# HyTruongSon/GraphFlow

Measured on AMD Instinct MI355X. Metric: CCN-2D (SMP_omega) molecules/sec fwd+bwd, higher is better.
Workload: dtype f32 (level block products: 2xf16-split operands, 22-bit, fp32 accumulate); 1 GPU; cfg3: SMP_omega 3 levels, C=64, F=5, D=5, cap=29, batch=1024 synthetic QM9-size molecules/GPU, device-resident, fused levels; parallelism=single GPU

## Files before the change

graphflow_amd/_lib.py:

```python
import ctypes as C
import os
import subprocess

_CSRC = os.path.join(os.path.dirname(os.path.abspath(__file__)), "csrc")
LIB_PATH = os.environ.get("GF_HIP_LIBRARY") or os.path.join(_CSRC, "libgf_hip.so")

GF_OK, GF_ERR_INVALID, GF_ERR_HIP, GF_ERR_NOMEM, GF_ERR_UNSUPPORTED, GF_ERR_TIMEOUT = range(6)
GF_OPT_R18_GENERIC_KERNELS = 1
GF_OPT_SMP_FP32_PRODUCTS = 2
GF_DIST_ID_BYTES = 128

_fp = C.POINTER(C.c_float)
_dp = C.POINTER(C.c_double)
_vp = C.c_void_p

PROTOTYPES = {
    "gf_ctx_create": (C.c_int, [C.POINTER(_vp), C.c_int, _vp]),
    "gf_ctx_use_private_stream": (C.c_int, [_vp]),
    "gf_ctx_destroy": (C.c_int, [_vp]),
    "gf_ctx_set_stream": (C.c_int, [_vp, _vp]),
    "gf_ctx_get_stream": (_vp, [_vp]),
    "gf_ctx_synchronize": (C.c_int, [_vp]),
    "gf_ctx_reserve": (C.c_int, [_vp, C.c_size_t]),
    "gf_ctx_set_timing": (C.c_int, [_vp, C.c_int]),
# ... 70 lines not shown
    "gf_smp_parameters_upload": (_i, [_vp, _fp]),
    "gf_smp_parameters_download": (_i, [_vp, _fp, _fp]),
    "gf_smp_forward_host": (_i, [_vp, _dp, _dp, _dp, _dp]),
    "gf_smp_adam_step": (_i, [_vp, _vp, _vp, C.c_double, _i]),
    "gf_smp_adam_reset": (_i, [_vp]),
    "gf_smp_momentum_step": (_i, [_vp, _vp, _vp, C.c_double, _i, C.c_double]),
    "gf_smp_uniform_init_host": (_i, [_vp, _fp]),
    "gf_smp_save_model": (_i, [_vp, _vp, C.c_char_p]),
    "gf_smp_load_model": (_i, [_vp, _vp, C.c_char_p]),
    "gf_smp_set_fused": (_i, [_vp, _i]),
    "gf_smp_device_bytes": (_i, [_vp, _vp, _vp]),
    "gf_smp_level_products_f32": (_i, [_vp, _i, _i, _vp, _vp, _vp, _vp, _vp]),
    "gf_smp_level_wgrad_f32": (_i, [_vp, _i, _vp, _vp, _vp, _vp, _vp]),
    "gf_smp_level_products_ex_f32": (_i, [_vp, _i, _i, _i, _i, _i, _vp, _vp, _vp, _vp, _vp, _vp, _i, _vp]),
    "gf_smp_level_wgrad_ex_f32": (_i, [_vp, _i, _i, _i, _i, _vp, _vp, _vp, _vp, _vp, _vp, _vp]),
    "gf_smp_prepare_molecule_host": (_i, [_vp, _i, C.POINTER(C.c_int), _dp, C.POINTER(C.c_int), _dp]),
    "gf_smp_receptive_field": (_i, [_vp, _i, _i, _i, C.POINTER(C.c_int), _i]),
    "gf_smp_read_activation": (C.c_longlong, [_vp, _i, _i, _i, _vp, C.c_size_t]),
    "gf_smp_read_reduced_adjacency": (C.c_longlong, [_vp, _i, _i, _i, _vp, C.c_size_t]),
    "gf_smp_level_sizes": (_i, [_vp, _i, C.POINTER(C.c_longlong), C.POINTER(C.c_longlong), C.POINTER(C.c_longlong)]),
    "gf_smp_level_present_rows": (C.c_longlong, [_vp, _i]),
    "gf_smp_level_pairs": (C.c_longlong, [_vp, _i]),
    "gf_smp_level_covered_rows": (C.c_longlong, [_vp, _i]),
    "gf_stack_forward_f32": (_i, [_vp, _vp, _vp, _i, C.c_size_t]),
    "gf_stack_backward_f32": (_i, [_vp, _vp, _vp, _i, C.c_size_t]),
})

PROTOTYPES.update({
    "gf_smp_dropout_masks": (_i, [_vp, _vp, C.c_float]),
    "gf_adam_step_f32": (_i, [_vp, _vp, _vp, _vp, _vp, C.c_size_t, C.c_double, _i, C.c_ulonglong]),
# ... 40 lines not shown
```

graphflow_amd/csrc/smp_fused.hip:

```cpp
#include <algorithm>
#include <type_traits>

#include "r18_device.h"
#include "smp_internal.h"

using namespace gf::dev;

namespace gf {
namespace {

__device__ __forceinline__ f4 fold_two_tables(f4 u, f4 v) {
    f4 z;
#pragma unroll
    for (int k = 0; k < 4; ++k) {
        const auto r = __builtin_amdgcn_permlane16_swap(__float_as_uint(u[k]), __float_as_uint(v[k]), false, false);
        z[k] = xor32_sum(__uint_as_float(r[0]) + __uint_as_float(r[1]));
    }
    return z;
}

__device__ __forceinline__ f4 dpp_xor8(f4 v) {
    f4 r;
#pragma unroll
    for (int k = 0; k < 4; ++k)
// ... 1423 lines not shown
    }
    const int ocols = smp_compact_o(s) ? 2 : O_COLS;
    const int ldt = T_COLS * C, ldo = O_COLS * C;
    {
        const long long tC = C, wCC = (long long)CC;
        GemmSpec sp[3] = {
            {T, d.Wst, O + O_LOC * C, rows, C, 5 * C, ldt, C, ldo, 3, {T_SAB * tC, T_SAB * tC, T_T6 * tC, 0}, {0 * wCC, 2 * wCC, 3 * wCC, 0},
             {2 * C, C, 2 * C, 0}, d.rowscale, 2, {0, 1, -1, -1}},
            {T + T_SAB * C, d.Wst + 5 * CC, O + O_Z * C, rows, C, 2 * C, ldt, C, ldo, 0, {0, 0, 0, 0}, {0, 0, 0, 0}, {0, 0, 0, 0}, nullptr, 0,
             {-1, -1, -1, -1}},
            {T + T_SAB * C, d.Wst + 7 * CC, O + O_ZP * C, rows, C, C, ldt, C, ldo, 0, {0, 0, 0, 0}, {0, 0, 0, 0}, {0, 0, 0, 0}, nullptr, 0,
             {-1, -1, -1, -1}},
        };
        if (smp_c64_kernels(s)) {
            st = smp_rowpanel_products_c64(ctx, true, T, drop ? d.rowfac8 : d.rowscale, d.Wst, O, rows, d.trow, d.trowf, false,
                                           d.wimg_ready ? d.wimg : nullptr, C, drop ? 8 : 2, smp_extras_in_kernel(s, l) ? 3 : 0);
            if (st != GF_OK) return st;
        } else if (gemm_grouped_supported(sp, 3, false, false)) {
            st = gemm_grouped_rows(ctx, false, false, sp, 3, rows);
            if (st != GF_OK) return st;
        } else {
            struct G { int tcol, kb, wpos, ocol, scol, acc; };
            const G gs[5] = {{T_SAB, 2, 0, O_LOC, 0, 0}, {T_SAB, 1, 2, O_LOC, 1, 1}, {T_T6, 2, 3, O_LOC, -1, 1},
                             {T_SAB, 2, 5, O_Z, -1, 0}, {T_SAB, 1, 7, O_ZP, -1, 0}};
            for (const G &g : gs) {
                st = gemm_rs(ctx, false, false, rows, C, g.kb * C, T + g.tcol * C, ldt, 0, d.Wst + g.wpos * CC, C, 0, O + g.ocol * C, ldo,
                             0, 1, g.acc, d.rowscale, 2, g.scol);
                if (st != GF_OK) return st;
            }
        }
    }
// ... 217 lines not shown
        fa.splits[g] = grp[g]->splits;
        fa.n[g] = (unsigned)grp[g]->n;
        fa.first[g] = firsts[g];
    }
    fa.part[5] = colpart;
    fa.splits[5] = nb;
    fa.n[5] = (unsigned)C;
    fa.first[5] = firsts[5];
    const unsigned total = (unsigned)(18 * CC + C);
    GF_LAUNCH(ctx, "smpf_fold", smp_fold_level, dim3((total + 63) / 64), dim3(256), 0, fa, dKl, dbl, C, s->cfg.custom_matmul, total);
    st = smp_dp_level_done(s, l);
    if (st != GF_OK) return st;
    if (d.fwd_c64) {
        st = smp_rowpanel_products_c64(ctx, false, dO, drop ? d.rowfac8 : d.rowscale, d.Wst, dT, rows, ocols == 2 ? d.trow : nullptr, d.trowf,
                                       smp_fused_gather_enabled(s, l), d.wimg_ready ? d.wimg : nullptr, C, drop ? 8 : 2,
                                       (ocols == 2 && smp_extras_in_kernel(s, l)) ? 3 : 0);
        x_bwd_done = ocols == 2 && smp_extras_in_kernel(s, l);
        if (st != GF_OK) return st;
    } else {
        const long long oC = C, wCC = (long long)CC;
        GemmSpec dg[3] = {
            {dO, d.Wst, dT + T_SAB * C, rows, C, 4 * C, ldo, C, ldt, 4, {O_LOC * oC, O_LOC * oC, O_Z * oC, O_ZP * oC},
             {0 * wCC, 2 * wCC, 5 * wCC, 7 * wCC}, {C, C, C, C}, d.rowscale, 2, {0, 1, -1, -1}},
            {dO, d.Wst, dT + T_SBC * C, rows, C, 2 * C, ldo, C, ldt, 2, {O_LOC * oC, O_Z * oC, 0, 0}, {1 * wCC, 6 * wCC, 0, 0}, {C, C, 0, 0},
             d.rowscale, 2, {0, -1, -1, -1}},
            {dO, d.Wst, dT + T_T6 * C, rows, 2 * C, C, ldo, C, ldt, 1, {O_LOC * oC, 0, 0, 0}, {3 * wCC, 0, 0, 0}, {C, 0, 0, 0}, nullptr, 0,
             {-1, -1, -1, -1}},
        };
        if (gemm_grouped_supported(dg, 3, false, true)) {
            st = gemm_grouped_rows(ctx, false, true, dg, 3, rows);
            if (st != GF_OK) return st;
// ... 187 lines not shown
```

graphflow_amd/csrc/smp_internal.h:

```cpp
#ifndef GF_SMP_INTERNAL_H_INCLUDED
#define GF_SMP_INTERNAL_H_INCLUDED

#include <vector>

#include "gf_internal.h"
#include "smp_prep.h"

namespace gf {
gf_status gemm(gf_ctx *ctx, bool ta, bool tb, int M, int N, int K, const float *A, int lda, long long sA, const float *B,
               int ldb, long long sB, float *C, int ldc, long long sC, int batch, int accumulate);
gf_status gemm_rs(gf_ctx *ctx, bool ta, bool tb, int M, int N, int K, const float *A, int lda, long long sA, const float *B,
                  int ldb, long long sB, float *C, int ldc, long long sC, int batch, int accumulate, const float *rs,
                  int rs_ld, int scol);
struct GemmSpec {
    const float *A, *B;
    float *C;
    int M, N, K, lda, ldb, ldc;
    int nseg;
    long long a_off[4], b_off[4];
    int klen[4];
    const float *rs;
    int rs_ld;
    int scol[4];
};
struct FoldGroup {
    const float *part;
    int splits;
    size_t n;
};
gf_status gemm_grouped_free(gf_ctx *ctx, bool tb, const GemmSpec *specs, int n, const char *name);
gf_status gemm_grouped_free_tn(gf_ctx *ctx, const GemmSpec *specs, int n, float *part, size_t part_floats, FoldGroup *out,
                               const char *name);
bool gemm_grouped_supported(const GemmSpec *specs, int n, bool ta, bool tb);
gf_status gemm_grouped_rows(gf_ctx *ctx, bool ta, bool tb, const GemmSpec *specs, int n, int rows, int accumulate = 0);
gf_status gemm_grouped_splitk(gf_ctx *ctx, const GemmSpec *specs, int n, int rows, float *dest, int accumulate);
gf_status smp_rowpanel_products_c64(gf_ctx *ctx, bool forward, const float *A, const float *rowscale, const float *Wst, float *Out,
                                    int rows, const int *trow, const int *trowf = nullptr, bool skip_zero_grads = false,
                                    const void *wimg = nullptr, int C = 64,
                                    int nf = 2, int nx = 0);
bool smp_split_products(const gf_ctx *ctx);
gf_status smp_rowpanel_split_c64(gf_ctx *ctx, bool forward, const float *A, const float *rowscale, const float *Wst, float *Out,
                                 int rows, const int *trow, int cus, const int *trowf = nullptr, bool skip_zero_grads = false,
                                 const void *wimg = nullptr, int C = 64, int nf = 2, int nx = 0);
size_t smp_split_image_bytes();
gf_status smp_split_build_images(gf_ctx *ctx, const float *const *Wst, void *const *img, int n, int C = 64, const float *const *X = nullptr);
gf_status smp_wgrad_partials_all(gf_ctx *ctx, const float *T, const float *dO, const float *rowscale, int rows, int splits, float *part,
                                 const int *trow, const int *trowf, unsigned *words, const unsigned *chan = nullptr, float smax = 0.f,
                                 const unsigned *row_max = nullptr, int nf = 2, int C = 32, float *xpart = nullptr);
gf_status smp_wgrad_channel_maxima_ld(gf_ctx *ctx, const float *fprev, long long prev_rows, int ld0, const float *dsrc, long long drows, int ld1, int C,
                                      unsigned *words);
size_t smp_wgrad_all_words();
int smp_wgrad_all_splits(gf_ctx *ctx, long long rows);
gf_status smp_small_split_c64(gf_ctx *ctx, bool transposed, int n, const int *prog, const float *const *In, float *const *Out, const int *rows,
                              const int *pos0, const void *wimg, const char *name, int C = 64);
struct WgradScales {
    const unsigned *cmax = nullptr, *chan = nullptr;
    float smax = 0.f, max_tot = 0.f, max_tr = 0.f;
    const unsigned *row_max = nullptr;
// ... 71 lines not shown
        int4 *tf_recs = nullptr;
        float *psum = nullptr;
        float *dshl = nullptr;
        bool psum_ready = false;
        float *pmax = nullptr;
        float *dzmax = nullptr;
        long long dz_rows = 0;
        int dz_ld = 64;
        long long dz_rows2 = 0, dz_off2 = 0;
        int dz_ld2 = 64;
        bool pmax_ready = false;
        void *wimg = nullptr;
        bool wimg_ready = false;
        bool fwd_c64 = false;
        int *trowf = nullptr;
        float max_tot = 0.f, max_tr = 0.f;
        const unsigned *row_max = nullptr;
        long long *pair_src_pair = nullptr, *cons_row = nullptr, *cons_pair = nullptr;
        int *node_center = nullptr, *cons_a = nullptr, *mol_order = nullptr, *gather_items = nullptr;
        float *Fdc = nullptr, *Gc = nullptr, *dGc = nullptr, *dFdc = nullptr;
        float *f = nullptr, *df = nullptr, *Q = nullptr;
        float *sh = nullptr, *vf = nullptr;
        int *node_of_vertex = nullptr, *node_mol = nullptr;
        int *node_present = nullptr;
        int *field = nullptr;
        unsigned *keep_mask = nullptr;
        float *nodefac = nullptr, *rowfac8 = nullptr;
        float *Vt = nullptr, *dVt = nullptr;
        float *St = nullptr, *dSt = nullptr;
        float *scal = nullptr;
// ... 121 lines not shown
```

graphflow_amd/csrc/smp_level_c64.hip:

```cpp
#include <algorithm>
#include <cstdlib>

#include "gemm_lds.h"
#include "gf_internal.h"
#include "smp_internal.h"

namespace gf {
namespace {

using namespace lds_image;

constexpr int kWgThreads = 1024, kWgARows = 256, kWgBRows = 192;
constexpr int kWgStage = (kWgARows + kWgBRows) * LDS_ROW + 2 * BK;
__constant__ int c_wg_ablk[8] = {0, 1, 0, 2, 3, 0, 1, 0};
__constant__ int c_wg_bblk[8] = {0, 0, 0, 0, 0, 1, 1, 2};
__constant__ int c_wg_scale[8] = {0, 0, 1, -1, -1, -1, -1, -1};

__global__ __launch_bounds__(kWgThreads, 1) void smp_wgrad_c64(const float *__restrict__ T, const float *__restrict__ dO,
                                                               const float *__restrict__ rs, int rows, int kchunk,
                                                               float *__restrict__ part, const int *__restrict__ trow) {
    extern __shared__ __attribute__((aligned(16))) float wg_smem[];
    const int tid = threadIdx.x, lane = tid & 63, li = lane & 31, lh = lane >> 5;
    const int wave = __builtin_amdgcn_readfirstlane(tid >> 6);
    const int prod = wave >> 1, nh = wave & 1;
// ... 350 lines not shown
    if (kchunk < 8 * BK) kchunk = 8 * BK;
    const int splits = (rows + kchunk - 1) / kchunk;
    if ((size_t)splits * total > part_floats)
        return fail(ctx, GF_ERR_NOMEM, "smp_wgrad_partials_c64: %d partial images, room for %zu", splits, part_floats / total);
    out->splits = splits;
    if (trow && ws.any() && smp_split_products(ctx))
        return smp_wgrad_partials_split_c64(ctx, T, dO, rowscale, rows, kchunk, splits, part, trow, ws, trowf);
    const size_t lds = sizeof(float) * 2 * (size_t)kWgStage;
    gf_status st = opt_in_lds(ctx, smp_wgrad_c64, lds);
    if (st != GF_OK) return st;
    GF_LAUNCH(ctx, "smpf_wgrad", smp_wgrad_c64, dim3((unsigned)splits), dim3(kWgThreads), lds, T, dO, rowscale, rows, kchunk, part, trow);
    return GF_OK;
}

gf_status smp_rowpanel_products_c64(gf_ctx *ctx, bool forward, const float *A, const float *rowscale, const float *Wst, float *Out,
                                    int rows, const int *trow, const int *trowf, bool skip_zero_grads, const void *wimg, int C, int nf, int nx) {
    if (rows < 1) return GF_OK;
    static int cu_count[64] = {};
    const int di = ctx->device & 63;
    if (!cu_count[di]) {
        GF_HIP_TRY(ctx, hipDeviceGetAttribute(&cu_count[di], hipDeviceAttributeMultiprocessorCount, ctx->device));
        if (cu_count[di] < 1) cu_count[di] = 256;
    }
    const int cus = cu_count[di];
    if (trow && smp_split_products(ctx)) return smp_rowpanel_split_c64(ctx, forward, A, rowscale, Wst, Out, rows, trow, cus, trowf, skip_zero_grads, wimg, C, nf, nx);
    if (C != 64 || nf != 2 || nx != 0) return fail(ctx, GF_ERR_UNSUPPORTED, "smp_rowpanel_products: %d channels / %d row factors / %d extra products on the fp32 matrix pipe", C, nf, nx);
    const size_t lds = sizeof(float) * 8 * 2 * 2 * 32 * (size_t)kRpWRow;
    const int th = (forward && !trow) ? 1024 : 512;
    const int npanels = (rows + 31) / 32, per = th / 64;
    const int want = (npanels + per - 1) / per;
    const int grid = want < cus ? want : cus;
    const char *name = forward ? "smpf_products_fwd" : "smpf_products_bwd";
#define GF_RP_LAUNCH(F, T, Cm)                                                                                              \
    do {                                                                                                                    \
        gf_status st__ = opt_in_lds(ctx, smp_rowpanel_c64<F, T, Cm>, lds);                                                  \
        if (st__ != GF_OK) return st__;                                                                                     \
        GF_LAUNCH(ctx, name, (smp_rowpanel_c64<F, T, Cm>), dim3((unsigned)grid), dim3(T), lds, A, rowscale, Wst, Out, rows, trow); \
    } while (0)
    if (trow) {
        if (forward) GF_RP_LAUNCH(true, 512, true);
// ... 12 lines not shown
```

graphflow_amd/csrc/smp_level_c64_split.hip:

```cpp
#include <cstdlib>
#include <type_traits>

#include "gemm_lds.h"
#include "gf_internal.h"
#include "smp_internal.h"

namespace gf {
namespace {

using lds_image::f16v;
using lds_image::f4v;
typedef _Float16 h8 __attribute__((ext_vector_type(8)));
typedef _Float16 h2 __attribute__((ext_vector_type(2)));
typedef float f2v __attribute__((ext_vector_type(2)));

constexpr int kSpThreads = 512;

template <unsigned EMIN = 14u>
__device__ __forceinline__ void pow2_scale(unsigned maxbits, float *s, float *inv) {
    unsigned e = maxbits >> 23;
    e = e < EMIN ? EMIN : e;
    *s = __uint_as_float((267u - e) << 23);
    *inv = __uint_as_float((e - 13u) << 23);
}
// ... 81 lines not shown
        if (blockIdx.x == 0)
            build_weight_images<true, 1, 16>(w, H, L, winv, wmax, threadIdx.x);
        else
            build_weight_images<false, 1, 16>(w, H, L, winv, wmax, threadIdx.x);
    } else {
        if (blockIdx.x == 0)
            build_weight_images<true, 1, 32>(w, H, L, winv, wmax, threadIdx.x);
        else
            build_weight_images<false, 1, 32>(w, H, L, winv, wmax, threadIdx.x);
    }
}

#ifndef GF_SP_WHOLE_PANEL
#define GF_SP_WHOLE_PANEL 16
#endif
template <bool FWD, bool MASK, int CB = 64, int NF = 2, int NX = 0>
__global__ __launch_bounds__(kSpThreads, 1) void smp_rowpanel_split(const float *__restrict__ A, const float *__restrict__ rs,
                                                                     const float *__restrict__ Wst, float *__restrict__ Out, int rows,
                                                                     const int *__restrict__ trow, int store_mask,
                                                                     const uint4 *__restrict__ wimg) {
    constexpr int LDA = FWD ? 4 * CB : 2 * CB, LDOUT = FWD ? 2 * CB : 4 * CB;
    constexpr int VPL = CB / 2, NC = CB / 16, NH = CB >= 32 ? CB / 32 : 1, E = NH * NC * 64;
    auto t_row = [](int t) { return MASK ? (t & 0x1fffffff) : t; };
    auto t_own = [](int t) { return MASK ? t < 0 : true; };
    auto t_tr = [](int t) { return MASK ? ((t >> 30) & 1) != 0 : true; };
    auto t_bc = [](int t) { return MASK ? ((t >> 29) & 1) != 0 : true; };
    static_assert(NX == 0 || (NX == 3 && CB <= 32 && NF == 2), "the extra products: prebuilt images, plain row factors");
    constexpr int NP = 8 + NX;
    extern __shared__ __attribute__((aligned(16))) uint4 sp_smem[];
    uint4 *imgH = sp_smem, *imgL = sp_smem + NP * E;
    float *winv = reinterpret_cast<float *>(sp_smem + 2 * NP * E);
    unsigned *wmax = reinterpret_cast<unsigned *>(winv + 16);
    float *facs = winv + 32;
    const int tid = threadIdx.x, lane = tid & 63, li = lane & 31, lh = lane >> 5;
    const int wave = tid >> 6;

    if (wimg) {
        for (int t = tid; t < NP * E; t += kSpThreads) {
            const int pos = t / E, g = (pos < 8 ? pos : kSpStacked + pos - 8) * 512 + t % E;
            imgH[t] = wimg[g];
            imgL[t] = wimg[kSpAll + g];
        }
        if (tid < 2) reinterpret_cast<uint4 *>(winv)[tid] = wimg[2 * kSpAll + tid];
        if (NX > 0 && tid < NX) winv[8 + tid] = reinterpret_cast<const float *>(wimg + 2 * kSpAll)[kSpStacked + tid];
    } else {
        static_assert(E == 512 || true, "");
        if constexpr (CB == 64) build_weight_images<FWD, 8>(Wst, imgH, imgL, winv, wmax, tid);
    }
    __syncthreads();

// ... 137 lines not shown
                if constexpr (NH == 2) gf_st_s<2>(out + (size_t)rr * LDOUT + 32, acc1[r]);
            }
        } else {
            const unsigned mine = (MASK && !FWD) ? rowbits >> (4 * lh) : 0xffffffffu;
#pragma unroll
            for (int r = 0; r < 16; ++r) {
                const int rr = (r & 3) + 8 * (r >> 2);
                if (r0 + 4 * lh + rr < rows && li < CB && ((mine >> rr) & 1u)) {
                    gf_st_s<2>(out + (size_t)rr * LDOUT, acc0[r]);
                    if constexpr (NH == 2) gf_st_s<2>(out + (size_t)rr * LDOUT + 32, acc1[r]);
                }
            }
        }
    };

    int tnext = fetch_trow(blockIdx.x * (kSpThreads / 64) + wave);
    auto panel = [&](int p, Raw &Ra, Raw &Rb, auto full) {
        const int pn = p + nwaves;
        const int tcur = tnext;
        tnext = fetch_trow(pn);
        const RowFac sc = load_scale(p);
        f16v acc0, acc1;
        Spl X, Y, Z;
        float iX, iY, iZ;
        if (FWD) {
            split_blk(Ra, X, iX);
            load_raw(Ra, p, 1, t_bc(tcur));
            split_blk(Rb, Z, iZ);
            load_raw(Rb, p, 2, t_own(tcur));
            clear(acc0, acc1);
            prod(X, iX * sc.f[5], 5, acc0, acc1);
// ... 37 lines not shown
            }
            store_out(p, 1, acc0, acc1, full);
            load_raw_at(Ra, t_row(tcur), 1, !(MASK && store_mask) || t_own(tcur));
            load_raw(Rb, pn, 1, !(MASK && store_mask) || t_bc(tnext));
            clear(acc0, acc1);
            prod(X, iX * sc.f[0], 0, acc0, acc1);
            prod(X, iX * sc.f[2], 2, acc0, acc1);
            prod(Y, iY * sc.f[5], 5, acc0, acc1);
            if constexpr (NX == 3) prod(X, iX, 8, acc0, acc1);
            split_blk(Ra, Z, iZ);
            load_raw(Ra, pn, 0, !(MASK && store_mask) || t_bc(tnext));
            prod(Z, iZ * sc.f[7], 7, acc0, acc1);
            store_out(p, 0, acc0, acc1, full, rowbits);
        }
    };
    if constexpr (CB <= GF_SP_WHOLE_PANEL) {
        constexpr int NB = FWD ? 5 : 3;
        Raw R[NB];
        int p = blockIdx.x * (kSpThreads / 64) + wave;
        int t1 = tnext, t2 = fetch_trow(p + nwaves);
        auto request = [&](int q, int t) {
            if constexpr (FWD) {
                load_raw(R[0], q, 0, t_own(t));
                load_raw_at(R[1], t_row(t), 0, t_tr(t));
                load_raw(R[2], q, 1, t_bc(t));
                load_raw(R[3], q, 2, t_own(t));
                load_raw(R[4], q, 3, t_bc(t));
            } else {
                const bool all = !(MASK && store_mask);
                load_raw(R[0], q, 0, all || t_bc(t));
// ... 826 lines not shown
        }
        GF_LAUNCH(ctx, "smpf_stack_w", smp_split_weight_images, dim3(2, m, kSpPos), dim3(kSpThreads), 0, a, C);
    }
    return GF_OK;
}

struct RowpanelArgs {
    int grid;
    const float *A, *rowscale, *Wst;
    float *Out;
    int rows;
    const int *trow;
    int store_mask;
    const uint4 *img;
};
template <bool F, bool M, int CB, int NF, int NX>
static gf_status launch_rowpanel_split(gf_ctx *ctx, const RowpanelArgs &a) {
    const size_t lds = 2 * (size_t)(8 + NX) * (CB >= 32 ? CB / 32 : 1) * (CB / 16) * 64 * 16 + 32 * sizeof(float) + (kSpThreads / 64) * 32 * sizeof(float);
    gf_status st = opt_in_lds(ctx, smp_rowpanel_split<F, M, CB, NF, NX>, lds);
    if (st != GF_OK) return st;
    GF_LAUNCH(ctx, F ? "smpf_products_fwd" : "smpf_products_bwd", (smp_rowpanel_split<F, M, CB, NF, NX>), dim3((unsigned)a.grid), dim3(kSpThreads),
              lds, a.A, a.rowscale, a.Wst, a.Out, a.rows, a.trow, a.store_mask, a.img);
    return GF_OK;
}
template <int CB, int NF, int NX = 0>
static gf_status launch_rowpanel_split(gf_ctx *ctx, bool forward, bool mask, const RowpanelArgs &a) {
    if (forward) return mask ? launch_rowpanel_split<true, true, CB, NF, NX>(ctx, a) : launch_rowpanel_split<true, false, CB, NF, NX>(ctx, a);
    return mask ? launch_rowpanel_split<false, true, CB, NF, NX>(ctx, a) : launch_rowpanel_split<false, false, CB, NF, NX>(ctx, a);
}

gf_status smp_rowpanel_split_c64(gf_ctx *ctx, bool forward, const float *A, const float *rowscale, const float *Wst, float *Out,
                                 int rows, const int *trow, int cus, const int *trowf, bool skip_zero_grads, const void *wimg, int C, int nf, int nx) {
    const int per = kSpThreads / 64;
    const int npanels = (rows + 31) / 32;
    const int want = (npanels + per - 1) / per;
    const int slots = C == 64 ? cus : 2 * cus;
    const int grid = want < slots ? want : slots;
    if (C != 64 && !wimg) return fail(ctx, GF_ERR_UNSUPPORTED, "smp_rowpanel_split: %d channels need the level's prebuilt weight images", C);
    const bool mask = packed_rows(trowf, rows, 1 << 29);
    const RowpanelArgs a = {grid, A, rowscale, Wst, Out, rows, mask ? trowf : trow, skip_zero_grads ? 1 : 0,
                            wimg ? static_cast<const uint4 *>(wimg) + (forward ? 0 : kSpImgStride) : nullptr};
    if (nx != 0) {
        if (nx != 3 || nf != 2 || !(C == 32 || C == 16) || !wimg)
            return fail(ctx, GF_ERR_UNSUPPORTED, "smp_rowpanel_split: %d extra products at %d channels / %d row factors", nx, C, nf);
        return C == 32 ? launch_rowpanel_split<32, 2, 3>(ctx, forward, mask, a) : launch_rowpanel_split<16, 2, 3>(ctx, forward, mask, a);
    }
    if (nf != 2 && !(nf == 8 && (C == 32 || C == 16))) return fail(ctx, GF_ERR_UNSUPPORTED, "smp_rowpanel_split: %d row factors at %d channels", nf, C);
    if (nf == 8)
        return C == 32 ? launch_rowpanel_split<32, 8>(ctx, forward, mask, a) : launch_rowpanel_split<16, 8>(ctx, forward, mask, a);
    switch (C) {
    case 64: return launch_rowpanel_split<64, 2>(ctx, forward, mask, a);
    case 32: return launch_rowpanel_split<32, 2>(ctx, forward, mask, a);
    case 16: return launch_rowpanel_split<16, 2>(ctx, forward, mask, a);
    }
    return fail(ctx, GF_ERR_UNSUPPORTED, "smp_rowpanel_split: %d channels", C);
}

gf_status smp_wgrad_partials_split_c64(gf_ctx *ctx, const float *T, const float *dO, const float *rowscale, int rows, int kchunk,
                                       int splits, float *part, const int *trow, const WgradScales &ws, const int *trowf) {
    gf_status st = opt_in_lds(ctx, smp_wgrad_split, kWsLds);
    if (st != GF_OK) return st;
    const bool mask = packed_rows(trowf, rows, 1 << 29);
    GF_LAUNCH(ctx, "smpf_wgrad", smp_wgrad_split, dim3((unsigned)splits), dim3(kWsThreads), kWsLds, T, dO, rowscale, rows, kchunk, part,
              mask ? trowf : trow, ws.cmax, ws.chan, ws.smax, ws.max_tot, ws.max_tr, ws.row_max, mask ? 1 : 0);
    return GF_OK;
}
// ... 91 lines not shown
```

graphflow_amd/csrc/smp_level_ops.hip:

```cpp
#include <cstring>
#include <vector>

#include "smp_internal.h"

using gf::fail;

namespace gf {
namespace {

__global__ __launch_bounds__(256) void rowfac8_absmax(const float *__restrict__ rf, int rows, unsigned *__restrict__ out) {
    float a = 1.f, b = 0.f, c = 1.f;
    for (int r = blockIdx.x * blockDim.x + threadIdx.x; r < rows; r += gridDim.x * blockDim.x) {
        const float *f = rf + 8 * (size_t)r;
        a = fmaxf(a, fmaxf(fmaxf(fabsf(f[0]), fabsf(f[1])), fmaxf(fabsf(f[5]), fmaxf(fabsf(f[6]), fabsf(f[7])))));
        b = fmaxf(b, fabsf(f[2]));
        c = fmaxf(c, fmaxf(fabsf(f[3]), fabsf(f[4])));
    }
    atomicMax(&out[0], __float_as_uint(a));
    atomicMax(&out[1], __float_as_uint(b));
    atomicMax(&out[2], __float_as_uint(c));
}
__global__ void scale_words(unsigned *__restrict__ w, int n, const unsigned *__restrict__ by) {
    const int i = blockIdx.x * blockDim.x + threadIdx.x;
    if (i < n) w[i] = __float_as_uint(__uint_as_float(w[i]) * __uint_as_float(by[0]));
// ... 65 lines not shown
}

gf_status gf_smp_level_products_ex_f32(gf_ctx *ctx, int backward, int C, int nf, int nx, int rows, const float *A, const float *rowfac,
                                       const float *Wst, const float *X, const int *trow, const int *trowf, int skip_zero_grads, float *Out) {
    static const char *who = "gf_smp_level_products_ex_f32";
    if (!ctx) return fail(nullptr, GF_ERR_INVALID, "null context");
    if (rows < 0 || (rows > 0 && (!A || !rowfac || !Wst || !trow || !Out))) return fail(ctx, GF_ERR_INVALID, "%s: null argument", who);
    if (nx == 3 && !X) return fail(ctx, GF_ERR_INVALID, "%s: three extra products without their weight blocks", who);
    gf_status st = gf::check_variant(ctx, who, C, nf, nx, true);
    if (st != GF_OK) return st;
    if (rows == 0) return GF_OK;
    GF_HIP_TRY(ctx, hipSetDevice(ctx->device));
    st = gf::check_tables(ctx, who, rows, trow, trowf, 0);
    if (st != GF_OK) return st;
    void *img = nullptr;
    if (gf::smp_split_products(ctx)) {
        const size_t CC = (size_t)C * C, img_bytes = gf::align_up(gf::smp_split_image_bytes(), 256);
        st = gf::ensure_ws(ctx, img_bytes + sizeof(float) * 18 * CC + 256);
        if (st != GF_OK) return st;
        img = ctx->ws;
        float *w18 = reinterpret_cast<float *>(static_cast<char *>(ctx->ws) + img_bytes);
        GF_HIP_TRY(ctx, hipMemcpyAsync(w18, Wst, sizeof(float) * 8 * CC, hipMemcpyDeviceToDevice, ctx->stream));
        GF_HIP_TRY(ctx, hipMemsetAsync(w18 + 8 * CC, 0, sizeof(float) * 10 * CC, ctx->stream));
        const float *wp = w18, *xp = nx == 3 ? X : nullptr;
        st = gf::smp_split_build_images(ctx, &wp, &img, 1, C, &xp);
        if (st != GF_OK) return st;
    }
    return gf::smp_rowpanel_products_c64(ctx, backward == 0, A, rowfac, Wst, Out, rows, trow, trowf, skip_zero_grads != 0, img, C, nf, nx);
}

gf_status gf_smp_level_wgrad_ex_f32(gf_ctx *ctx, int C, int nf, int nx, int rows, const float *T, const float *dO, const float *rowfac,
                                    const int *trow, const int *trowf, float *dWst, float *dX) {
    static const char *who = "gf_smp_level_wgrad_ex_f32";
    if (!ctx) return fail(nullptr, GF_ERR_INVALID, "null context");
    if (rows < 1 || !T || !dO || !rowfac || !trow || !dWst) return fail(ctx, GF_ERR_INVALID, "%s: bad argument", who);
    if (nx == 3 && !dX) return fail(ctx, GF_ERR_INVALID, "%s: three extra products without a place for their gradients", who);
    gf_status st = gf::check_variant(ctx, who, C, nf, nx, false);
    if (st != GF_OK) return st;
    GF_HIP_TRY(ctx, hipSetDevice(ctx->device));
    st = gf::check_tables(ctx, who, rows, trow, trowf, gf::kGatherWindow);
    if (st != GF_OK) return st;
    const size_t CC = (size_t)C * C;
    const int splits = gf::smp_wgrad_all_splits(ctx, rows);
// ... 26 lines not shown
```

graphflow_amd/csrc/smp_prepare.hip:

```cpp
#include <chrono>
#include <cmath>
#include <cstdio>
#include <cstdlib>

#include "smp_internal.h"

namespace gf {
void *pinned_table_alloc(size_t bytes) {
    void *p = nullptr;
    const size_t total = bytes + 16;
    unsigned kind = 1;
    if (hipHostMalloc(&p, total, hipHostMallocPortable) != hipSuccess) p = nullptr;
    if (!p) {
        (void)hipGetLastError();
        p = std::malloc(total);
        kind = 0;
        if (!p) return nullptr;
    }
    *static_cast<unsigned *>(p) = kind;
    return static_cast<char *>(p) + 16;
}
void pinned_table_free(void *q) {
    if (!q) return;
    void *p = static_cast<char *>(q) - 16;
// ... 317 lines not shown
        const int it = (i % s) * s + i / s;
        const long long t = r0 + it;
        trow[r0 + i] = (int)t;
        const bool own = pi[r0 + i] >= 0, tr = pi[r0 + it] >= 0;
        bool bc = false;
        {
            const int b = i / s, c = i % s;
            for (int a = 0; a < s && !bc; ++a) bc = pi[r0 + a * s + b] >= 0 && pi[r0 + a * s + c] >= 0;
        }
        rowflag[r0 + i] = (own ? 1 : 0) | (bc ? 2 : 0);
        if (trowf)
            trowf[r0 + i] = (t < (1ll << 29)) ? (int)((unsigned)t | (own ? 0x80000000u : 0u) | (tr ? 0x40000000u : 0u) | (bc ? 0x20000000u : 0u)) : -1;
    }
}

struct Taker {
    gf_smp *s;
    gf_status st = GF_OK;
    template <typename T>
    void alloc(T **p, size_t count) {
        if (st == GF_OK) st = upload(s, p, nullptr, count);
    }
    template <typename T, typename V>
    void put(T **p, const V &v) {
        if (st == GF_OK) st = upload(s, p, v.empty() ? nullptr : &v[0], v.size());
    }
    template <typename T, typename V>
    void table(T **p, const V &v, size_t count) {
        s->lay.device_tables ? alloc(p, count) : put(p, v);
    }
// ... 115 lines not shown

void alloc_level_gather(Taker &t, Level &h, DevLevel &d) {
    const gfsmp::Config &cfg = t.s->cfg;
    if (!(cfg.square() && cfg.nContractions == 18 && cfg.nChanels % 4 == 0 && t.s->bwd_gather)) return;
    t.alloc(&d.cons_hdr, (size_t)h.pairs * 2);
    t.alloc(&d.cons_qrec, (size_t)h.qrec_total);
    t.put(&d.cons_qbase, h.cons_qbase);
}

void alloc_level_panels(Taker &t, Level &h, DevLevel &d, int l) {
    const gfsmp::Config &cfg = t.s->cfg;
    const int L = cfg.nLevels, C = cfg.nChanels;
    if (!(cfg.square() && smp_panel_channels(C) && h.rows < 0x7fffffffll)) return;
    t.alloc(&d.trow, (size_t)h.rows);
    t.alloc(&d.trowf, (size_t)h.rows);
    unsigned char *img = nullptr;
    t.alloc(&img, smp_split_image_bytes());
    d.wimg = img;
    t.alloc(&d.rowflag, (size_t)h.rows);
    if (!(cfg.nContractions == 18 && h.rows * 256 < 0x3fffffffll && !h.buckets.empty() && h.buckets.back().s <= kFusedMaxField)) return;
    const int np = h.npanels;
    const size_t np1 = (size_t)(np > 0 ? np : 1);
    d.fwd_npanels = np;
    t.put(&d.node_panel, h.node_panel);
    t.alloc(&d.fwd_pan, np1);
    if (l == L || cfg.physics) t.alloc(&d.psum, np1 * C);
    if (l < L) t.alloc(&d.pmax, np1 * C);
    t.alloc(&d.dzmax, (h.quad_node.size() + np1) * 64);
    t.alloc(&d.fwd_pan_node, np1);
    t.alloc(&d.fwd_goff, (size_t)h.rows);
// ... 92 lines not shown

gf_status build_row_tables(gf_smp *s) {
    hipStream_t up = upload_stream(s);
    for (int l = 1; l <= s->cfg.nLevels; ++l) {
        const gf_smp::DevLevel &d = s->lv[l];
        const int nNodes = s->lay.level[l].nNodes;
        const bool merged = d.node_tables_merged;
        if (!merged)
            hipLaunchKernelGGL(expand_rowscale, dim3(nNodes), dim3(64), 0, up, reinterpret_cast<float2 *>(d.rowscale),
                               reinterpret_cast<const float2 *>(d.node_scale), d.node_s, d.node_row);
        gf_status st = smp_build_gather_records(s, l, up);
        if (st == GF_OK) st = smp_build_tf_records(s, l, up);
        if (st == GF_OK) st = smp_fwd_fused_build_tables(s, l, up, !merged);
        if (st != GF_OK) return st;
        if (d.trow && !merged) hipLaunchKernelGGL(build_trow, dim3(nNodes), dim3(64), 0, up, d.trow, d.node_s, d.node_row, d.pi, d.rowflag, d.trowf);
    }
    return GF_OK;
}

gf_status alloc_readout(gf_smp *s, int nMol) {
    const gfsmp::BatchLayout &B = s->lay;
    const int L = s->cfg.nLevels, C = s->cfg.nChanels;
    const gfsmp::LevelLayout &top = B.level[L];
    Taker t = {s};
    t.put(&s->x, B.x);
    s->wbound = nullptr;
    if (s->cfg.square() && C == 64) t.alloc(&s->wbound, smp_wgrad_bound_words() * (size_t)(L + 1));
    else if (s->cfg.square() && (C == 32 || C == 16))
        t.alloc(&s->wbound, smp_wgrad_all_words() * (size_t)(L + 1));
    t.alloc(&s->sh, (size_t)top.nNodes * C);
// ... 11 lines not shown
    }
    t.put(&s->top_node_mol, top.node_mol);
    t.put(&s->mol_ptr, B.mol_first_vertex);
    t.put(&s->mol_nodes, B.top_node_of_vertex);
    long long maxrows = 0, maxpairs = 0;
    for (int l = 0; l <= L; ++l) {
        maxrows = std::max(maxrows, (long long)B.level[l].rows);
        maxpairs = std::max(maxpairs, (long long)B.level[l].pairs);
    }
    s->colpart_rows = (size_t)((maxrows + 1023) / 1024 + (maxpairs + 255) / 256 + 2);
    s->colpart_rows = std::max(s->colpart_rows, (size_t)256 * (L + 1));
    t.alloc(&s->colpart, s->colpart_rows * C);
    return t.st;
}

}
}

using gf::fail;

extern "C" {

gf_status gf_smp_prepare(gf_smp *s, int nMol, const int *nVertices, const int *adj, const double *feature) {
    return gf_smp_prepare_coulomb(s, nMol, nVertices, adj, feature, nullptr);
}

gf_status gf_smp_prepare_coulomb(gf_smp *s, int nMol, const int *nVertices, const int *adj, const double *feature,
                                 const double *coulomb) {
    if (!s) return fail(nullptr, GF_ERR_INVALID, "null smp handle");
    gf_ctx *ctx = s->ctx;
// ... 66 lines not shown
```

include/gf_hip.h:

```cpp
#ifndef GF_HIP_H_INCLUDED
#define GF_HIP_H_INCLUDED

#include <stddef.h>

#ifdef __cplusplus
extern "C" {
#endif

typedef struct gf_ctx gf_ctx;

typedef enum {
    GF_OK = 0,
    GF_ERR_INVALID = 1,
    GF_ERR_HIP = 2,
    GF_ERR_NOMEM = 3,
    GF_ERR_UNSUPPORTED = 4,
    GF_ERR_TIMEOUT = 5
} gf_status;

gf_status gf_ctx_create(gf_ctx **out, int device, void *stream);
gf_status gf_ctx_use_private_stream(gf_ctx *ctx);
gf_status gf_ctx_destroy(gf_ctx *ctx);
gf_status gf_ctx_set_stream(gf_ctx *ctx, void *stream);
void     *gf_ctx_get_stream(gf_ctx *ctx);
// ... 122 lines not shown
size_t    gf_head_work_floats(int nLayers, const int *width, int n);
gf_status gf_head_forward_f32(gf_ctx *ctx, int nLayers, const int *width, const float *x, int n, const float *params,
                              const float *targets, float *predict, float *loss, float *work);
gf_status gf_head_backward_f32(gf_ctx *ctx, int nLayers, const int *width, const float *x, int n, const float *params, float *work,
                               float *dx, float *dparams);
gf_status gf_smp_set_fused(gf_smp *smp, int on);
gf_status gf_smp_level_products_f32(gf_ctx *ctx, int backward, int rows, const float *A, const float *rowscale, const float *Wst,
                                    const int *trow, float *Out);
gf_status gf_smp_level_wgrad_f32(gf_ctx *ctx, int rows, const float *T, const float *dO, const float *rowscale, const int *trow,
                                 float *dWst);
gf_status gf_smp_level_products_ex_f32(gf_ctx *ctx, int backward, int C, int nf, int nx, int rows, const float *A, const float *rowfac,
                                       const float *Wst, const float *X, const int *trow, const int *trowf, int skip_zero_grads,
                                       float *Out);
gf_status gf_smp_level_wgrad_ex_f32(gf_ctx *ctx, int C, int nf, int nx, int rows, const float *T, const float *dO, const float *rowfac,
                                    const int *trow, const int *trowf, float *dWst, float *dX);
gf_status gf_smp_device_bytes(const gf_smp *smp, size_t *in_use, size_t *reserved);
gf_status gf_smp_parameters_upload(gf_smp *smp, const float *host_params);
gf_status gf_smp_parameters_download(gf_smp *smp, float *host_params, float *host_grads);
gf_status gf_smp_forward_host(gf_smp *smp, const double *targets, double *predict, double *loss, double *graph_feature);
gf_status gf_smp_adam_step(gf_smp *smp, float *params, const float *grads, double learning_rate, int nBatch);
gf_status gf_smp_adam_reset(gf_smp *smp);
gf_status gf_smp_momentum_step(gf_smp *smp, float *params, const float *grads, double learning_rate, int nBatch, double gamma);
gf_status gf_smp_uniform_init_host(const gf_smp_config *cfg, float *params);
gf_status gf_smp_classifier_uniform_init_host(const gf_smp_config *cfg, int nClass, float *params);
gf_status gf_smp_save_model(const gf_smp *smp, const float *params, const char *path);
gf_status gf_smp_load_model(gf_smp *smp, float *params, const char *path);
gf_status gf_smp_prepare_molecule_host(const gf_smp_config *cfg, int V, const int *adj, const double *feature,
                                       int *phi_out, double *wl_out);
int       gf_smp_receptive_field(const gf_smp *smp, int mol, int level, int v, int *out, int capacity);
long long gf_smp_read_activation(gf_smp *smp, int mol, int level, int v, float *host_out, size_t capacity);
// ... 37 lines not shown
```

Measured before the change: 153,600 molecules/s.

## Partition backward product rows into own/absent classes to skip unneeded products

Adds a device-side compaction (count, scan, fill kernels) that splits the rows of each level into two lists: rows with their own entry and rows without one. It builds these lists once at table-preparation time. A new specialised backward split-products kernel walks the own rows with the full set of products, then walks the absent rows doing only the two products they need, writing through per-row pointers held in LDS. The aim is to stop masked-off work and divergence in the masked backward pass, at the cost of extra preprocessing kernels, more LDS, and scattered stores.

Measured after the change: 156,000 molecules/s (median of 6 runs). 1.02x the previous value.

```diff
diff --git a/graphflow_amd/_lib.py b/graphflow_amd/_lib.py
--- a/graphflow_amd/_lib.py
+++ b/graphflow_amd/_lib.py
@@ -108,6 +108,7 @@
     "gf_smp_level_wgrad_f32": (_i, [_vp, _i, _vp, _vp, _vp, _vp, _vp]),
     "gf_smp_level_products_ex_f32": (_i, [_vp, _i, _i, _i, _i, _i, _vp, _vp, _vp, _vp, _vp, _vp, _i, _vp]),
     "gf_smp_level_wgrad_ex_f32": (_i, [_vp, _i, _i, _i, _i, _vp, _vp, _vp, _vp, _vp, _vp, _vp]),
+    "gf_smp_level_row_classes": (_i, [_vp, _i, _vp, _vp]),
     "gf_smp_prepare_molecule_host": (_i, [_vp, _i, C.POINTER(C.c_int), _dp, C.POINTER(C.c_int), _dp]),
     "gf_smp_receptive_field": (_i, [_vp, _i, _i, _i, C.POINTER(C.c_int), _i]),
     "gf_smp_read_activation": (C.c_longlong, [_vp, _i, _i, _i, _vp, C.c_size_t]),
diff --git a/graphflow_amd/csrc/smp_fused.hip b/graphflow_amd/csrc/smp_fused.hip
--- a/graphflow_amd/csrc/smp_fused.hip
+++ b/graphflow_amd/csrc/smp_fused.hip
@@ -1461,7 +1461,7 @@
         };
         if (smp_c64_kernels(s)) {
             st = smp_rowpanel_products_c64(ctx, true, T, drop ? d.rowfac8 : d.rowscale, d.Wst, O, rows, d.trow, d.trowf, false,
-                                           d.wimg_ready ? d.wimg : nullptr, C, drop ? 8 : 2, smp_extras_in_kernel(s, l) ? 3 : 0);
+                                           d.wimg_ready ? d.wimg : nullptr, C, drop ? 8 : 2, smp_extras_in_kernel(s, l) ? 3 : 0, d.rowcls);
             if (st != GF_OK) return st;
         } else if (gemm_grouped_supported(sp, 3, false, false)) {
             st = gemm_grouped_rows(ctx, false, false, sp, 3, rows);
@@ -1709,7 +1709,7 @@
     if (d.fwd_c64) {
         st = smp_rowpanel_products_c64(ctx, false, dO, drop ? d.rowfac8 : d.rowscale, d.Wst, dT, rows, ocols == 2 ? d.trow : nullptr, d.trowf,
                                        smp_fused_gather_enabled(s, l), d.wimg_ready ? d.wimg : nullptr, C, drop ? 8 : 2,
-                                       (ocols == 2 && smp_extras_in_kernel(s, l)) ? 3 : 0);
+                                       (ocols == 2 && smp_extras_in_kernel(s, l)) ? 3 : 0, d.rowcls);
         x_bwd_done = ocols == 2 && smp_extras_in_kernel(s, l);
         if (st != GF_OK) return st;
     } else {
diff --git a/graphflow_amd/csrc/smp_internal.h b/graphflow_amd/csrc/smp_internal.h
--- a/graphflow_amd/csrc/smp_internal.h
+++ b/graphflow_amd/csrc/smp_internal.h
@@ -37,11 +37,14 @@
 gf_status smp_rowpanel_products_c64(gf_ctx *ctx, bool forward, const float *A, const float *rowscale, const float *Wst, float *Out,
                                     int rows, const int *trow, const int *trowf = nullptr, bool skip_zero_grads = false,
                                     const void *wimg = nullptr, int C = 64,
-                                    int nf = 2, int nx = 0);
+                                    int nf = 2, int nx = 0,
+                                    const int *rowcls = nullptr);
 bool smp_split_products(const gf_ctx *ctx);
 gf_status smp_rowpanel_split_c64(gf_ctx *ctx, bool forward, const float *A, const float *rowscale, const float *Wst, float *Out,
                                  int rows, const int *trow, int cus, const int *trowf = nullptr, bool skip_zero_grads = false,
-                                 const void *wimg = nullptr, int C = 64, int nf = 2, int nx = 0);
+                                 const void *wimg = nullptr, int C = 64, int nf = 2, int nx = 0, const int *rowcls = nullptr);
+size_t smp_row_class_ints(int rows);
+gf_status smp_build_row_classes(gf_ctx *ctx, hipStream_t stream, const int *trowf, int rows, int *buf);
 size_t smp_split_image_bytes();
 gf_status smp_split_build_images(gf_ctx *ctx, const float *const *Wst, void *const *img, int n, int C = 64, const float *const *X = nullptr);
 gf_status smp_wgrad_partials_all(gf_ctx *ctx, const float *T, const float *dO, const float *rowscale, int rows, int splits, float *part,
@@ -143,6 +146,7 @@
         bool wimg_ready = false;
         bool fwd_c64 = false;
         int *trowf = nullptr;
+        int *rowcls = nullptr;
         float max_tot = 0.f, max_tr = 0.f;
         const unsigned *row_max = nullptr;
         long long *pair_src_pair = nullptr, *cons_row = nullptr, *cons_pair = nullptr;
diff --git a/graphflow_amd/csrc/smp_level_c64.hip b/graphflow_amd/csrc/smp_level_c64.hip
--- a/graphflow_amd/csrc/smp_level_c64.hip
+++ b/graphflow_amd/csrc/smp_level_c64.hip
@@ -388,7 +388,8 @@
 }
 
 gf_status smp_rowpanel_products_c64(gf_ctx *ctx, bool forward, const float *A, const float *rowscale, const float *Wst, float *Out,
-                                    int rows, const int *trow, const int *trowf, bool skip_zero_grads, const void *wimg, int C, int nf, int nx) {
+                                    int rows, const int *trow, const int *trowf, bool skip_zero_grads, const void *wimg, int C, int nf, int nx,
+                                    const int *rowcls) {
     if (rows < 1) return GF_OK;
     static int cu_count[64] = {};
     const int di = ctx->device & 63;
@@ -397,7 +398,7 @@
         if (cu_count[di] < 1) cu_count[di] = 256;
     }
     const int cus = cu_count[di];
-    if (trow && smp_split_products(ctx)) return smp_rowpanel_split_c64(ctx, forward, A, rowscale, Wst, Out, rows, trow, cus, trowf, skip_zero_grads, wimg, C, nf, nx);
+    if (trow && smp_split_products(ctx)) return smp_rowpanel_split_c64(ctx, forward, A, rowscale, Wst, Out, rows, trow, cus, trowf, skip_zero_grads, wimg, C, nf, nx, rowcls);
     if (C != 64 || nf != 2 || nx != 0) return fail(ctx, GF_ERR_UNSUPPORTED, "smp_rowpanel_products: %d channels / %d row factors / %d extra products on the fp32 matrix pipe", C, nf, nx);
     const size_t lds = sizeof(float) * 8 * 2 * 2 * 32 * (size_t)kRpWRow;
     const int th = (forward && !trow) ? 1024 : 512;
diff --git a/graphflow_amd/csrc/smp_level_c64_split.hip b/graphflow_amd/csrc/smp_level_c64_split.hip
--- a/graphflow_amd/csrc/smp_level_c64_split.hip
+++ b/graphflow_amd/csrc/smp_level_c64_split.hip
@@ -119,11 +119,13 @@
 #ifndef GF_SP_WHOLE_PANEL
 #define GF_SP_WHOLE_PANEL 16
 #endif
-template <bool FWD, bool MASK, int CB = 64, int NF = 2, int NX = 0>
+template <bool FWD, bool MASK, int CB = 64, int NF = 2, int NX = 0, bool CLS = false>
 __global__ __launch_bounds__(kSpThreads, 1) void smp_rowpanel_split(const float *__restrict__ A, const float *__restrict__ rs,
                                                                      const float *__restrict__ Wst, float *__restrict__ Out, int rows,
                                                                      const int *__restrict__ trow, int store_mask,
-                                                                     const uint4 *__restrict__ wimg) {
+                                                                     const uint4 *__restrict__ wimg,
+                                                                     const int *__restrict__ rcls) {
+    static_assert(!CLS || (!FWD && MASK && CB == 64 && NF == 2 && NX == 0), "row classes: the masked backward products at 64 channels");
     constexpr int LDA = FWD ? 4 * CB : 2 * CB, LDOUT = FWD ? 2 * CB : 4 * CB;
     constexpr int VPL = CB / 2, NC = CB / 16, NH = CB >= 32 ? CB / 32 : 1, E = NH * NC * 64;
     auto t_row = [](int t) { return MASK ? (t & 0x1fffffff) : t; };
@@ -139,6 +141,8 @@
     float *facs = winv + 32;
     const int tid = threadIdx.x, lane = tid & 63, li = lane & 31, lh = lane >> 5;
     const int wave = tid >> 6;
+    typedef unsigned long long u64x2 __attribute__((ext_vector_type(2)));
+    unsigned long long *rowp = reinterpret_cast<unsigned long long *>(facs + (kSpThreads / 64) * 32);
 
     if (wimg) {
         for (int t = tid; t < NP * E; t += kSpThreads) {
@@ -306,7 +310,7 @@
         }
     };
 
-    int tnext = fetch_trow(blockIdx.x * (kSpThreads / 64) + wave);
+    int tnext = CLS ? 0 : fetch_trow(blockIdx.x * (kSpThreads / 64) + wave);
     auto panel = [&](int p, Raw &Ra, Raw &Rb, auto full) {
         const int pn = p + nwaves;
         const int tcur = tnext;
@@ -374,6 +378,101 @@
             store_out(p, 0, acc0, acc1, full, rowbits);
         }
     };
+    if constexpr (CLS) {
+        const int n_own_p = (rcls[0] + 31) >> 5, n_tot_p = n_own_p + ((rcls[1] + 31) >> 5), n_ent = 32 * n_tot_p;
+        const int2 *ent = reinterpret_cast<const int2 *>(rcls + 4);
+        unsigned long long *myrow = rowp + wave * 32;
+        auto fetch_entry = [&](int q, int *rw) {
+            const int i = q * 32 + li;
+            const int2 e = ent[i < n_ent ? i : n_ent - 1];
+            *rw = e.x;
+            return e.y;
+        };
+        auto e_row = [](int rw) { return rw & 0x1fffffff; };
+        auto scale_at = [&](int row) {
+            const float2 t = *reinterpret_cast<const float2 *>(rs + (size_t)row * 2);
+            RowFac r;
+            r.f[0] = r.f[1] = t.x, r.f[2] = t.y;
+            r.f[3] = r.f[4] = r.f[5] = r.f[6] = r.f[7] = 1.f;
+            return r;
+        };
+        auto post_rows = [&](int rw) {
+            __builtin_amdgcn_wave_barrier();
+            myrow[li] = reinterpret_cast<unsigned long long>(rw < 0 ? sp_dump + li * 64 : Out + (size_t)e_row(rw) * LDOUT);
+            __builtin_amdgcn_wave_barrier();
+        };
+        auto store_rows = [&](int o, const f16v &acc0, const f16v &acc1) {
+#pragma unroll
+            for (int g = 0; g < 4; ++g) {
+                const u64x2 a = *reinterpret_cast<const u64x2 *>(myrow + 8 * g + 4 * lh), b = *reinterpret_cast<const u64x2 *>(myrow + 8 * g + 4 * lh + 2);
+#pragma unroll
+                for (int j = 0; j < 4; ++j) {
+                    float *dst = reinterpret_cast<float *>(j < 2 ? a[j & 1] : b[j & 1]) + o * CB + li;
+                    gf_st_s<2>(dst, acc0[4 * g + j]);
+                    gf_st_s<2>(dst + 32, acc1[4 * g + j]);
+                }
+            }
+        };
+        int p = blockIdx.x * (kSpThreads / 64) + wave;
+        int rnext, tn = fetch_entry(p, &rnext);
+        Raw Ra, Rb;
+        load_raw_at(Rb, e_row(rnext), 1, t_bc(tn));
+        load_raw_at(Ra, e_row(rnext), 0, t_bc(tn));
+        auto panel_own = [&](int q) {
+            const int qn = q + nwaves, rcur = rnext, tcur = tn;
+            tn = fetch_entry(qn, &rnext);
+            const RowFac sc = scale_at(e_row(rcur));
+            post_rows(rcur);
+            f16v acc0, acc1;
+            Spl X, Y, Z;
+            float iX, iY, iZ;
+            split_blk(Ra, X, iX);
+            split_blk(Rb, Y, iY);
+            clear(acc0, acc1);
+            prod(X, iX * sc.f[3], 3, acc0, acc1);
+            store_rows(2, acc0, acc1);
+            clear(acc0, acc1);
+            prod(X, iX * sc.f[4], 4, acc0, acc1);
+            store_rows(3, acc0, acc1);
+            clear(acc0, acc1);
+            prod(X, iX * sc.f[1], 1, acc0, acc1);
+            prod(Y, iY * sc.f[6], 6, acc0, acc1);
+            store_rows(1, acc0, acc1);
+            load_raw_at(Ra, t_row(tcur), 1, t_own(tcur));
+            load_raw_at(Rb, e_row(rnext), 1, t_bc(tn));
+            clear(acc0, acc1);
+            prod(X, iX * sc.f[0], 0, acc0, acc1);
+            prod(X, iX * sc.f[2], 2, acc0, acc1);
+            prod(Y, iY * sc.f[5], 5, acc0, acc1);
+            split_blk(Ra, Z, iZ);
+            load_raw_at(Ra, e_row(rnext), 0, t_bc(tn));
+            prod(Z, iZ * sc.f[7], 7, acc0, acc1);
+            store_rows(0, acc0, acc1);
+        };
+        auto panel_absent = [&](int q) {
+            const int qn = q + nwaves, rcur = rnext;
+            tn = fetch_entry(qn, &rnext);
+            const RowFac sc = scale_at(e_row(rcur));
+            post_rows(rcur);
+            f16v acc0, acc1;
+            Spl X, Y;
+            float iX, iY;
+            split_blk(Ra, X, iX);
+            split_blk(Rb, Y, iY);
+            load_raw_at(Rb, e_row(rnext), 1, t_bc(tn));
+            load_raw_at(Ra, e_row(rnext), 0, t_bc(tn));
+            clear(acc0, acc1);
+            prod(X, iX * sc.f[4], 4, acc0, acc1);
+            store_rows(3, acc0, acc1);
+            clear(acc0, acc1);
+            prod(X, iX * sc.f[1], 1, acc0, acc1);
+            prod(Y, iY * sc.f[6], 6, acc0, acc1);
+            store_rows(1, acc0, acc1);
+        };
+        for (; p < n_own_p; p += nwaves) panel_own(p);
+        for (; p < n_tot_p; p += nwaves) panel_absent(p);
+        return;
+    }
     if constexpr (CB <= GF_SP_WHOLE_PANEL) {
         constexpr int NB = FWD ? 5 : 3;
         Raw R[NB];
@@ -1230,13 +1329,14 @@
     int store_mask;
     const uint4 *img;
 };
-template <bool F, bool M, int CB, int NF, int NX>
-static gf_status launch_rowpanel_split(gf_ctx *ctx, const RowpanelArgs &a) {
-    const size_t lds = 2 * (size_t)(8 + NX) * (CB >= 32 ? CB / 32 : 1) * (CB / 16) * 64 * 16 + 32 * sizeof(float) + (kSpThreads / 64) * 32 * sizeof(float);
-    gf_status st = opt_in_lds(ctx, smp_rowpanel_split<F, M, CB, NF, NX>, lds);
+template <bool F, bool M, int CB, int NF, int NX, bool CLS = false>
+static gf_status launch_rowpanel_split(gf_ctx *ctx, const RowpanelArgs &a, const int *rcls = nullptr) {
+    const size_t lds = 2 * (size_t)(8 + NX) * (CB >= 32 ? CB / 32 : 1) * (CB / 16) * 64 * 16 + 32 * sizeof(float) + (kSpThreads / 64) * 32 * sizeof(float) +
+                       (CLS ? (kSpThreads / 64) * 32 * sizeof(float *) : 0);
+    gf_status st = opt_in_lds(ctx, smp_rowpanel_split<F, M, CB, NF, NX, CLS>, lds);
     if (st != GF_OK) return st;
-    GF_LAUNCH(ctx, F ? "smpf_products_fwd" : "smpf_products_bwd", (smp_rowpanel_split<F, M, CB, NF, NX>), dim3((unsigned)a.grid), dim3(kSpThreads),
-              lds, a.A, a.rowscale, a.Wst, a.Out, a.rows, a.trow, a.store_mask, a.img);
+    GF_LAUNCH(ctx, F ? "smpf_products_fwd" : "smpf_products_bwd", (smp_rowpanel_split<F, M, CB, NF, NX, CLS>), dim3((unsigned)a.grid), dim3(kSpThreads),
+              lds, a.A, a.rowscale, a.Wst, a.Out, a.rows, a.trow, a.store_mask, a.img, rcls);
     return GF_OK;
 }
 template <int CB, int NF, int NX = 0>
@@ -1246,9 +1346,12 @@
 }
 
 gf_status smp_rowpanel_split_c64(gf_ctx *ctx, bool forward, const float *A, const float *rowscale, const float *Wst, float *Out,
-                                 int rows, const int *trow, int cus, const int *trowf, bool skip_zero_grads, const void *wimg, int C, int nf, int nx) {
+                                 int rows, const int *trow, int cus, const int *trowf, bool skip_zero_grads, const void *wimg, int C, int nf, int nx,
+                                 const int *rowcls) {
     const int per = kSpThreads / 64;
-    const int npanels = (rows + 31) / 32;
+    const bool classed = rowcls && !forward && skip_zero_grads && C == 64 && nf == 2 && nx == 0 && packed_rows(trowf, rows, 1 << 29) &&
+                         !env_is("GF_SMP_ROW_CLASSES", '0');
+    const int npanels = (rows + 31) / 32 + (classed ? 1 : 0);
     const int want = (npanels + per - 1) / per;
     const int slots = C == 64 ? cus : 2 * cus;
     const int grid = want < slots ? want : slots;
@@ -1265,7 +1368,9 @@
     if (nf == 8)
         return C == 32 ? launch_rowpanel_split<32, 8>(ctx, forward, mask, a) : launch_rowpanel_split<16, 8>(ctx, forward, mask, a);
     switch (C) {
-    case 64: return launch_rowpanel_split<64, 2>(ctx, forward, mask, a);
+    case 64:
+        if (classed) return launch_rowpanel_split<false, true, 64, 2, 0, true>(ctx, a, rowcls);
+        return launch_rowpanel_split<64, 2>(ctx, forward, mask, a);
     case 32: return launch_rowpanel_split<32, 2>(ctx, forward, mask, a);
     case 16: return launch_rowpanel_split<16, 2>(ctx, forward, mask, a);
     }
diff --git a/graphflow_amd/csrc/smp_level_ops.hip b/graphflow_amd/csrc/smp_level_ops.hip
--- a/graphflow_amd/csrc/smp_level_ops.hip
+++ b/graphflow_amd/csrc/smp_level_ops.hip
@@ -103,10 +103,19 @@
     st = gf::check_tables(ctx, who, rows, trow, trowf, 0);
     if (st != GF_OK) return st;
     void *img = nullptr;
+    const int *rowcls = nullptr;
     if (gf::smp_split_products(ctx)) {
         const size_t CC = (size_t)C * C, img_bytes = gf::align_up(gf::smp_split_image_bytes(), 256);
-        st = gf::ensure_ws(ctx, img_bytes + sizeof(float) * 18 * CC + 256);
+        const size_t w_bytes = gf::align_up(sizeof(float) * 18 * CC, 256);
+        const bool classes = trowf && C == 64 && rows < (1 << 29);
+        st = gf::ensure_ws(ctx, img_bytes + w_bytes + (classes ? sizeof(int) * gf::smp_row_class_ints(rows) : 0) + 256);
         if (st != GF_OK) return st;
+        if (classes) {
+            int *buf = reinterpret_cast<int *>(static_cast<char *>(ctx->ws) + img_bytes + w_bytes);
+            st = gf::smp_build_row_classes(ctx, ctx->stream, trowf, rows, buf);
+            if (st != GF_OK) return st;
+            rowcls = buf;
+        }
         img = ctx->ws;
         float *w18 = reinterpret_cast<float *>(static_cast<char *>(ctx->ws) + img_bytes);
         GF_HIP_TRY(ctx, hipMemcpyAsync(w18, Wst, sizeof(float) * 8 * CC, hipMemcpyDeviceToDevice, ctx->stream));
@@ -115,7 +124,14 @@
         st = gf::smp_split_build_images(ctx, &wp, &img, 1, C, &xp);
         if (st != GF_OK) return st;
     }
-    return gf::smp_rowpanel_products_c64(ctx, backward == 0, A, rowfac, Wst, Out, rows, trow, trowf, skip_zero_grads != 0, img, C, nf, nx);
+    return gf::smp_rowpanel_products_c64(ctx, backward == 0, A, rowfac, Wst, Out, rows, trow, trowf, skip_zero_grads != 0, img, C, nf, nx, rowcls);
+}
+
+gf_status gf_smp_level_row_classes(gf_ctx *ctx, int rows, const int *trowf, int *lists) {
+    if (!ctx) return fail(nullptr, GF_ERR_INVALID, "null context");
+    if (rows < 1 || rows >= (1 << 29) || !trowf || !lists) return fail(ctx, GF_ERR_INVALID, "gf_smp_level_row_classes: bad argument");
+    GF_HIP_TRY(ctx, hipSetDevice(ctx->device));
+    return gf::smp_build_row_classes(ctx, ctx->stream, trowf, rows, lists);
 }
 
 gf_status gf_smp_level_wgrad_ex_f32(gf_ctx *ctx, int C, int nf, int nx, int rows, const float *T, const float *dO, const float *rowfac,
diff --git a/graphflow_amd/csrc/smp_prepare.hip b/graphflow_amd/csrc/smp_prepare.hip
--- a/graphflow_amd/csrc/smp_prepare.hip
+++ b/graphflow_amd/csrc/smp_prepare.hip
@@ -355,6 +355,57 @@
     }
 }
 
+constexpr int kRcBlock = 1024;
+__global__ __launch_bounds__(kRcBlock) void row_class_count(const int *__restrict__ trowf, int rows, int *__restrict__ blockcnt) {
+    const int r = blockIdx.x * kRcBlock + threadIdx.x;
+    const int n = __syncthreads_count(r < rows && trowf[r] < 0);
+    if (threadIdx.x == 0) blockcnt[blockIdx.x] = n;
+}
+__global__ __launch_bounds__(kRcBlock) void row_class_scan(int *__restrict__ blockcnt, int nb, int rows, int *__restrict__ hdr) {
+    __shared__ int part[kRcBlock];
+    const int tid = threadIdx.x, per = (nb + kRcBlock - 1) / kRcBlock;
+    const int i0 = tid * per < nb ? tid * per : nb, i1 = i0 + per < nb ? i0 + per : nb;
+    int sum = 0;
+    for (int i = i0; i < i1; ++i) sum += blockcnt[i];
+    part[tid] = sum;
+    __syncthreads();
+    for (int d = 1; d < kRcBlock; d <<= 1) {
+        const int v = tid >= d ? part[tid - d] : 0;
+        __syncthreads();
+        part[tid] += v;
+        __syncthreads();
+    }
+    int run = part[tid] - sum;
+    for (int i = i0; i < i1; ++i) {
+        const int c = blockcnt[i];
+        blockcnt[i] = run;
+        run += c;
+    }
+    if (tid == kRcBlock - 1) hdr[0] = part[tid], hdr[1] = rows - part[tid], hdr[2] = hdr[3] = 0;
+}
+__global__ __launch_bounds__(kRcBlock) void row_class_fill(const int *__restrict__ trowf, int rows, const int *__restrict__ blockoff,
+                                                           const int *__restrict__ hdr, int2 *__restrict__ ent) {
+    __shared__ int wcnt[kRcBlock / 64];
+    const int tid = threadIdx.x, lane = tid & 63, w = tid >> 6;
+    const int r = blockIdx.x * kRcBlock + tid;
+    const int t = r < rows ? trowf[r] : 0;
+    const bool own = t < 0;
+    const unsigned long long b = __ballot(own);
+    if (lane == 0) wcnt[w] = __popcll(b);
+    __syncthreads();
+    int before = blockoff[blockIdx.x] + __popcll(b & ((1ull << lane) - 1ull));
+    for (int i = 0; i < w; ++i) before += wcnt[i];
+    if (r >= rows) return;
+    const int n_own = hdr[0], n_abs = hdr[1], own_pad = (n_own + 31) & ~31;
+    const int k = own ? before : r - before;
+    const int at = own ? k : own_pad + k;
+    ent[at] = make_int2(r, t);
+    if (k == (own ? n_own : n_abs) - 1) {
+        const int end = own ? own_pad : own_pad + ((n_abs + 31) & ~31);
+        for (int i = at + 1; i < end; ++i) ent[i] = make_int2((int)((unsigned)r | 0x80000000u), t);
+    }
+}
+
 struct Taker {
     gf_smp *s;
     gf_status st = GF_OK;
@@ -500,6 +551,7 @@
     if (!(cfg.square() && smp_panel_channels(C) && h.rows < 0x7fffffffll)) return;
     t.alloc(&d.trow, (size_t)h.rows);
     t.alloc(&d.trowf, (size_t)h.rows);
+    if (C == 64 && cfg.nContractions == 18 && h.rows < (1ll << 29)) t.alloc(&d.rowcls, smp_row_class_ints((int)h.rows));
     unsigned char *img = nullptr;
     t.alloc(&img, smp_split_image_bytes());
     d.wimg = img;
@@ -622,6 +674,8 @@
         if (st == GF_OK) st = smp_fwd_fused_build_tables(s, l, up, !merged);
         if (st != GF_OK) return st;
         if (d.trow && !merged) hipLaunchKernelGGL(build_trow, dim3(nNodes), dim3(64), 0, up, d.trow, d.node_s, d.node_row, d.pi, d.rowflag, d.trowf);
+        if (d.rowcls) st = smp_build_row_classes(s->ctx, up, d.trowf, (int)s->lay.level[l].rows, d.rowcls);
+        if (st != GF_OK) return st;
     }
     return GF_OK;
 }
@@ -663,6 +717,18 @@
     return t.st;
 }
 
+}
+
+size_t smp_row_class_ints(int rows) { return 4 + 2 * ((size_t)rows + 64) + (size_t)(rows + kRcBlock - 1) / kRcBlock + 1; }
+gf_status smp_build_row_classes(gf_ctx *ctx, hipStream_t stream, const int *trowf, int rows, int *buf) {
+    if (rows < 1) return GF_OK;
+    const int nb = (rows + kRcBlock - 1) / kRcBlock;
+    int *blockcnt = buf + 4 + 2 * ((size_t)rows + 64);
+    hipLaunchKernelGGL(row_class_count, dim3(nb), dim3(kRcBlock), 0, stream, trowf, rows, blockcnt);
+    hipLaunchKernelGGL(row_class_scan, dim3(1), dim3(kRcBlock), 0, stream, blockcnt, nb, rows, buf);
+    hipLaunchKernelGGL(row_class_fill, dim3(nb), dim3(kRcBlock), 0, stream, trowf, rows, blockcnt, buf, reinterpret_cast<int2 *>(buf + 4));
+    GF_LAUNCH_CHECK(ctx, "row_class_fill");
+    return GF_OK;
 }
 }
 
diff --git a/include/gf_hip.h b/include/gf_hip.h
--- a/include/gf_hip.h
+++ b/include/gf_hip.h
@@ -160,6 +160,7 @@
                                        float *Out);
 gf_status gf_smp_level_wgrad_ex_f32(gf_ctx *ctx, int C, int nf, int nx, int rows, const float *T, const float *dO, const float *rowfac,
                                     const int *trow, const int *trowf, float *dWst, float *dX);
+gf_status gf_smp_level_row_classes(gf_ctx *ctx, int rows, const int *trowf, int *lists);
 gf_status gf_smp_device_bytes(const gf_smp *smp, size_t *in_use, size_t *reserved);
 gf_status gf_smp_parameters_upload(gf_smp *smp, const float *host_params);
 gf_status gf_smp_parameters_download(gf_smp *smp, float *host_params, float *host_grads);
```
